# SamuelGong/FLASHE

Hardware: AMD Instinct MI355X
Metric: ciphertexts/sec (enc+agg+dec), 1e7-elem vector; achieved HBM GB/s fraction (higher is better)
Workload: dtype u128

## Files before the change

flashe_amd/csrc/device_common.h:

```cpp
#pragma once
#include "kernels.h"

#include <algorithm>
#include <cstdlib>
#include <vector>

#ifdef FLASHE_TUNING
#define FLASHE_TUNE_ENV(name) getenv(name)
#else
#define FLASHE_TUNE_ENV(name) (static_cast<const char *>(nullptr))
#endif

namespace flashe {

typedef unsigned __int128 u128;
typedef __attribute__((address_space(3))) uint32_t lds_u32;
typedef __attribute__((address_space(3))) uint8_t lds_u8;
typedef uint64_t u64x2 __attribute__((ext_vector_type(2)));

constexpr int kTabWords = 32768;
constexpr int kIterShiftWord = 1024;
constexpr int kPrfThreads = 1024;

#define SEL_B0 0x0c020400u
// ... 260 lines not shown
__device__ __forceinline__ CtrPrefix scalar_prefix(const CtrPrefix &c)
{
    return CtrPrefix{{static_cast<uint32_t>(__builtin_amdgcn_readfirstlane(c.u[0])), static_cast<uint32_t>(__builtin_amdgcn_readfirstlane(c.u[1])),
                      static_cast<uint32_t>(__builtin_amdgcn_readfirstlane(c.u[2])), static_cast<uint32_t>(__builtin_amdgcn_readfirstlane(c.u[3]))}};
}

__device__ __forceinline__ CtrUniform ctr_uniform(const RoundKeys &rk, const uint32_t *__restrict__ te4, const CtrPrefix &c, uint32_t x3)
{
    const uint32_t S1 = c.u[1] ^ te4[512 + ((x3 >> 8) & 0xffu)];
    const uint32_t S2 = c.u[2] ^ te4[256 + ((x3 >> 16) & 0xffu)];
    const uint32_t S3 = c.u[3] ^ te4[x3 >> 24];
    CtrUniform r;
    r.u[0] = te4[256 + ((S1 >> 16) & 0xffu)] ^ te4[512 + ((S2 >> 8) & 0xffu)] ^ te4[768 + (S3 & 0xffu)] ^ rk.w[8];
    r.u[1] = te4[S1 >> 24] ^ te4[256 + ((S2 >> 16) & 0xffu)] ^ te4[512 + ((S3 >> 8) & 0xffu)] ^ rk.w[9];
    r.u[2] = te4[S2 >> 24] ^ te4[256 + ((S3 >> 16) & 0xffu)] ^ te4[768 + (S1 & 0xffu)] ^ rk.w[10];
    r.u[3] = te4[S3 >> 24] ^ te4[512 + ((S1 >> 8) & 0xffu)] ^ te4[768 + (S2 & 0xffu)] ^ rk.w[11];
    return r;
}

__device__ __forceinline__ void ctr_round2(const LaneRegs lr, uint32_t c0, uint32_t v0, const CtrUniform &U, uint32_t (&s)[4])
{
    const uint32_t s0 = c0 ^ v0;
    s[0] = U.u[0] ^ T0(s0, SEL_B3);
    s[1] = U.u[1] ^ T3(s0, SEL_B0);
    s[2] = U.u[2] ^ T2(s0, SEL_B1);
    s[3] = U.u[3] ^ T1(s0, SEL_B2);
}

__device__ __forceinline__ u128 words_to_u128(const uint32_t (&s)[4])
{
    const uint64_t hi = (static_cast<uint64_t>(s[0]) << 32) | s[1];
    const uint64_t lo = (static_cast<uint64_t>(s[2]) << 32) | s[3];
    return (static_cast<u128>(hi) << 64) | lo;
}

__device__ __forceinline__ void set_block(uint32_t (&s)[4], uint32_t iter, uint32_t idx, uint64_t ctr)
{
    s[0] = iter; s[1] = idx; s[2] = static_cast<uint32_t>(ctr >> 32); s[3] = static_cast<uint32_t>(ctr);
}

__device__ __forceinline__ u128 ld128(const uint64_t *p)
{
    const ulonglong2 v = *reinterpret_cast<const ulonglong2 *>(p);
    return (static_cast<u128>(v.y) << 64) | v.x;
}
__device__ __forceinline__ void st128(uint64_t *p, u128 v)
{
    *reinterpret_cast<ulonglong2 *>(p) = make_ulonglong2(static_cast<uint64_t>(v), static_cast<uint64_t>(v >> 64));
}

#define FLASHE_GLOBAL(T, p) (reinterpret_cast<__attribute__((address_space(1))) T *>(reinterpret_cast<uintptr_t>(p)))
__device__ __forceinline__ uint32_t ld32_g(const uint32_t *p) { return *FLASHE_GLOBAL(const uint32_t, p); }
__device__ __forceinline__ uint64_t ld64_g(const uint64_t *p) { return *FLASHE_GLOBAL(const uint64_t, p); }
__device__ __forceinline__ uint64_t ld64_nt_g(const uint64_t *p) { return __builtin_nontemporal_load(FLASHE_GLOBAL(const uint64_t, p)); }
__device__ __forceinline__ u128 ld128_g(const uint64_t *p)
{
    const u64x2 v = *FLASHE_GLOBAL(const u64x2, p);
    return (static_cast<u128>(v[1]) << 64) | v[0];
}
__device__ __forceinline__ u128 ld128_nt_g(const uint64_t *p)
{
    const u64x2 v = __builtin_nontemporal_load(FLASHE_GLOBAL(const u64x2, p));
    return (static_cast<u128>(v[1]) << 64) | v[0];
}
__device__ __forceinline__ void st128_nt_g(uint64_t *p, u128 v)
{
    u64x2 r;
    r[0] = static_cast<uint64_t>(v); r[1] = static_cast<uint64_t>(v >> 64);
    __builtin_nontemporal_store(r, FLASHE_GLOBAL(u64x2, p));
}

__device__ __forceinline__ u128 ld128_nt(const uint64_t *p)
{
    const u64x2 v = __builtin_nontemporal_load(reinterpret_cast<const u64x2 *>(p));
    return (static_cast<u128>(v[1]) << 64) | v[0];
}
__device__ __forceinline__ void st128_nt(uint64_t *p, u128 v)
{
    u64x2 r;
    r[0] = static_cast<uint64_t>(v); r[1] = static_cast<uint64_t>(v >> 64);
    __builtin_nontemporal_store(r, reinterpret_cast<u64x2 *>(p));
}


__device__ __forceinline__ double u128_to_double(u128 v)
{
    const uint64_t hi = static_cast<uint64_t>(v >> 64), lo = static_cast<uint64_t>(v);
    if (hi == 0) return static_cast<double>(lo);
    const int sh = 64 - __clzll(static_cast<long long>(hi));
    uint64_t m = static_cast<uint64_t>(v >> sh);
    const u128 dropped = v & ((static_cast<u128>(1) << sh) - 1);
    if (dropped) m |= 1;
    return ldexp(static_cast<double>(m), sh);
}

template <typename T>
__device__ __forceinline__ uint64_t quantize_one(T v, T alpha, T scale, T den, double u)
{
#pragma clang fp contract(off)
    v = v < -alpha ? -alpha : (v > alpha ? alpha : v);
    v = v + alpha;
    v = v * scale;
    v = v / den;
    return static_cast<uint64_t>(static_cast<int64_t>(floor(static_cast<double>(v) + u)));
}

__device__ __forceinline__ const CodecLayer *codec_layer_of(const Codec &c, uint64_t key)
{
    int lo = 0, hi = c.n_layers - 1;
    while (lo < hi) {
        const int mid = (lo + hi + 1) >> 1;
        if (c.layers[mid].start <= key) lo = mid; else hi = mid - 1;
    }
    return c.layers + lo;
}

__device__ __forceinline__ uint64_t codec_quantize(const Codec &c, uint64_t k)
{
    if (c.layers != nullptr) {
        const uint64_t key = c.k0 + k;
        const CodecLayer *L = codec_layer_of(c, key);
        const uint64_t r = key - L->start;
        return L->x_is_f64 ? quantize_one<double>(*FLASHE_GLOBAL(const double, static_cast<const double *>(L->x) + r), L->p0, L->p1, L->p2, c.u[k])
                           : quantize_one<float>(*FLASHE_GLOBAL(const float, static_cast<const float *>(L->x) + r), static_cast<float>(L->p0),
                                                 static_cast<float>(L->p1), static_cast<float>(L->p2), c.u[k]);
    }
    return c.x_is_f64 ? quantize_one<double>(static_cast<const double *>(c.x)[k], c.alpha, c.scale, c.den, c.u[k])
                      : quantize_one<float>(static_cast<const float *>(c.x)[k], static_cast<float>(c.alpha), static_cast<float>(c.scale),
                                            static_cast<float>(c.den), c.u[k]);
}

__device__ __forceinline__ double codec_unquantize(const Codec &c, uint64_t k, u128 v)
{
#pragma clang fp contract(off)
    if (c.layers != nullptr) {
        const CodecLayer *L = codec_layer_of(c, c.k0 + k);
        return u128_to_double(v) * L->p1 / L->p2 - L->p0;
    }
    return u128_to_double(v) * c.two_a / c.uden - c.ac;
}


static inline void masks_of(int b, uint64_t *lo, uint64_t *hi)
{
    if (b >= 128) { *lo = ~0ull; *hi = ~0ull; }
    else if (b > 64) { *lo = ~0ull; *hi = (1ull << (b - 64)) - 1; }
    else if (b == 64) { *lo = ~0ull; *hi = 0; }
    else { *lo = (1ull << b) - 1; *hi = 0; }
}

static inline int grid_for(const LaunchEnv &env, uint64_t work_items, int threads)
{
    uint64_t blocks = (work_items + threads - 1) / threads;
    if (blocks < 1) blocks = 1;
    if (blocks > static_cast<uint64_t>(env.num_cus)) blocks = env.num_cus;
    return static_cast<int>(blocks);
}


constexpr int kStreamThreads = 256;

static inline int stream_grid(const LaunchEnv &env, uint64_t items)
{
    uint64_t blocks = (items + kStreamThreads - 1) / kStreamThreads;
    const uint64_t cap = static_cast<uint64_t>(env.num_cus) * 8;
    if (blocks > cap) blocks = cap;
// ... 6 lines not shown
```

flashe_amd/csrc/kernels.hip:

```cpp
#include "device_common.h"

namespace flashe {

struct IdxLists {
    uint32_t add[kMaxIdx];
    uint32_t minus[kMaxIdx];
};

struct PrfParams {
    const uint64_t *in;
    uint64_t *out;
    const uint32_t *te0;
    uint64_t n;
    uint64_t first, count;
    uint64_t blk_first, blk_count;
    uint64_t mask_lo, mask_hi;
    uint32_t iter;
    int in_limbs;
    int n_add, n_minus;
    uint32_t n_jobs;
    int b, m;
    Codec cq;
};

__global__ __launch_bounds__(kPrfThreads) void prf_wide_kernel(const RoundKeys rk, const PrfParams p, const IdxLists lists)
{
    const uint32_t iter = p.iter + p.te0[kIterShiftWord];
    __shared__ uint32_t tab[kTabWords];
    fill_tables(tab, p.te0);
    const LaneRegs lr = lane_regs(tab);
    const u128 mask = (static_cast<u128>(p.mask_hi) << 64) | p.mask_lo;

    for (uint64_t base = static_cast<uint64_t>(blockIdx.x) * kPrfThreads; base < p.count;
         base += static_cast<uint64_t>(gridDim.x) * kPrfThreads) {
        const uint64_t e = base + threadIdx.x;
        if (e >= p.count) continue;
        const uint64_t j = p.first + e;
        u128 acc = 0;
        if (p.cq.x) acc = codec_quantize(p.cq, e);
        else if (p.in) acc = p.in_limbs == 2 ? ld128(p.in + 2 * e) : static_cast<u128>(p.in[e]);
        {
            int k = 0;
            for (; k + 1 < p.n_add; k += 2) {
                uint32_t s[2][4];
                set_block(s[0], iter, lists.add[k], j);
                set_block(s[1], iter, lists.add[k + 1], j);
                aes256_encrypt<2>(rk, lr, s);
                acc += words_to_u128(s[0]);
                acc += words_to_u128(s[1]);
            }
            if (k < p.n_add) {
                uint32_t s[1][4];
                set_block(s[0], iter, lists.add[k], j);
                aes256_encrypt<1>(rk, lr, s);
                acc += words_to_u128(s[0]);
            }
            k = 0;
            for (; k + 1 < p.n_minus; k += 2) {
                uint32_t s[2][4];
                set_block(s[0], iter, lists.minus[k], j);
                set_block(s[1], iter, lists.minus[k + 1], j);
                aes256_encrypt<2>(rk, lr, s);
                acc -= words_to_u128(s[0]);
                acc -= words_to_u128(s[1]);
            }
            if (k < p.n_minus) {
                uint32_t s[1][4];
                set_block(s[0], iter, lists.minus[k], j);
                aes256_encrypt<1>(rk, lr, s);
                acc -= words_to_u128(s[0]);
            }
        }
        if (p.cq.fout) p.cq.fout[e] = codec_unquantize(p.cq, e, acc & mask);
        else st128(p.out + 2 * e, acc & mask);
    }
}

struct JobTable {
    uint32_t add[kMaxBatch], minus[kMaxBatch];
    uint64_t first[kMaxBatch], count[kMaxBatch];
    uint64_t big_end[kMaxBatch], small_end[kMaxBatch];
    const uint64_t *in[kMaxBatch];
    uint64_t *out[kMaxBatch];
// ... 90 lines not shown
        uint64_t *sum_out = tb.sum_out_of(v);
        const bool uni = FLASHE_CTR2 && epl == kBigEpl && ctr_fast && ((first + kw) & 255u) == 0;
        CtrUniform Ua{}, Ub{};
        if (uni) {
            const uint32_t x3 = static_cast<uint32_t>(first + kw) ^ rk.w[3];
            Ua = ctr_uniform(rk, te0, pre_a, x3);
            if (DBL) Ub = ctr_uniform(rk, te0, pre_b, x3);
        }
        for (int e = 0; e < epl; e++) {
            const uint64_t k = kw + static_cast<uint64_t>(e) * 64u + lane;
            if (k >= count) break;
            const uint64_t j = first + k;
            u128 acc = !in ? static_cast<u128>(0) : in_limbs == 2 ? ld128(in + 2 * k) : static_cast<u128>(in[k]);
            u64x2 held[KIND == 2 ? kSumRegs : 1];
            if (KIND == 2 && n_in > 1) {
#pragma unroll
                for (int c = 0; c < kSumRegs; c++) {
                    const int cc = c + 1 < n_in ? c + 1 : 0;
                    held[c] = __builtin_nontemporal_load(reinterpret_cast<const u64x2 *>(in + static_cast<uint64_t>(cc) * in_stride + 2 * k));
                }
                for (int c = kSumRegs + 1; c < n_in; c++) acc += ld128_nt(in + static_cast<uint64_t>(c) * in_stride + 2 * k);
            }
            uint32_t s[DBL ? 2 : 1][4];
            if (uni) {
                const uint32_t v0 = T3(static_cast<uint32_t>(j) ^ rk.w[3], SEL_B0);
                ctr_round2(lr, pre_a.u[0], v0, Ua, s[0]);
                if (DBL) ctr_round2(lr, pre_b.u[0], v0, Ub, s[DBL ? 1 : 0]);
                aes256_rounds<DBL ? 2 : 1, 3>(rk, lr, s, true);
            } else if (ctr_fast) {
                const CtrVar x = ctr_var(rk, lr, static_cast<uint32_t>(j));
                ctr_round1(pre_a, x, s[0]);
                if (DBL) ctr_round1(pre_b, x, s[DBL ? 1 : 0]);
                aes256_rounds<DBL ? 2 : 1, 2>(rk, lr, s, true);
            } else {
                set_block(s[0], iter, ia, j);
                if (DBL) set_block(s[DBL ? 1 : 0], iter, im, j);
                aes256_encrypt<DBL ? 2 : 1>(rk, lr, s);
            }
            if (KIND == 2 && n_in > 1) {
#pragma unroll
                for (int c = 0; c < kSumRegs; c++)
                    if (c + 1 < n_in) acc += (static_cast<u128>(held[c][1]) << 64) | held[c][0];
                acc &= mask;
                if (sum_out) st128_nt(sum_out + 2 * k, acc);
            }
            acc += words_to_u128(s[0]);
            if (DBL) acc -= words_to_u128(s[DBL ? 1 : 0]);
            if (KIND == 2) st128_nt(out + 2 * k, acc & mask);
            else st128(out + 2 * k, acc & mask);
        }
    }
}

#ifndef FLASHE_HALF_U
#define FLASHE_HALF_U 1
#endif
constexpr int kMaxChains = 16;
constexpr int kMaxLinks = 128;
struct ChainTable {
    uint64_t first[kMaxChains], count[kMaxChains];
    uint64_t wend[kMaxChains];
    uint16_t link0[kMaxChains], sbase[kMaxChains];
    uint8_t len[kMaxChains];
    uint8_t flags[kMaxChains];
    uint32_t idx[kMaxLinks + kMaxChains];
    const uint64_t *in[kMaxLinks];
    uint64_t *out[kMaxLinks];
    uint64_t *sum_out[kMaxChains];
};

__device__ __forceinline__ CtrPrefix load_prefix(const uint32_t *pre_lds, int s)
{
    const uint4 v = *reinterpret_cast<const uint4 *>(pre_lds + 4 * s);
    return CtrPrefix{{static_cast<uint32_t>(__builtin_amdgcn_readfirstlane(v.x)), static_cast<uint32_t>(__builtin_amdgcn_readfirstlane(v.y)),
                      static_cast<uint32_t>(__builtin_amdgcn_readfirstlane(v.z)), static_cast<uint32_t>(__builtin_amdgcn_readfirstlane(v.w))}};
}

__device__ __forceinline__ void loads_landed(const u128 &a, const u128 &b)
{
    asm volatile("" ::"v"(static_cast<uint64_t>(a)), "v"(static_cast<uint64_t>(a >> 64)), "v"(static_cast<uint64_t>(b)),
                 "v"(static_cast<uint64_t>(b >> 64)));
}

template <class T> __device__ __forceinline__ void swap_regs(T &a, T &b) { const T t = a; a = b; b = t; }

__device__ __forceinline__ uint64_t uniform64(uint64_t v)
{
    return static_cast<uint32_t>(__builtin_amdgcn_readfirstlane(static_cast<uint32_t>(v))) |
           (static_cast<uint64_t>(static_cast<uint32_t>(__builtin_amdgcn_readfirstlane(static_cast<uint32_t>(v >> 32)))) << 32);
}

template <int THREADS, bool SUM, bool CODEC>
__global__ __launch_bounds__(THREADS) void prf_chain_kernel(const RoundKeys rk, const ChainTable tb, int n_chains, int all_half_arg,
                                                              uint32_t iter0, uint64_t mask_lo, uint64_t mask_hi,
                                                              const uint32_t *__restrict__ te0, const Codec cq)
{
    constexpr bool DMASK = false;
    uint64_t *const dmask = nullptr;
#include "prf_chain_body.inc"
}

template <int THREADS>
__global__ __launch_bounds__(THREADS) void prf_chain_dmask_kernel(const RoundKeys rk, const ChainTable tb, int n_chains, int all_half_arg,
                                                                    uint32_t iter0, uint64_t mask_lo, uint64_t mask_hi,
                                                                    const uint32_t *__restrict__ te0, uint64_t *__restrict__ dmask)
{
    constexpr bool SUM = true, CODEC = false, DMASK = true;
    const Codec cq{};
#include "prf_chain_body.inc"
}

__device__ __forceinline__ uint64_t extract64(u128 S, int sh)
{
    return sh >= 128 ? 0ull : static_cast<uint64_t>(S >> sh);
}

constexpr int kSmallThreads = 1024;
constexpr int kTch = 8;

__global__ __launch_bounds__(kSmallThreads) void prf_small_kernel(const RoundKeys rk, const PrfParams p, const IdxLists lists)
{
    const uint32_t iter = p.iter + p.te0[kIterShiftWord];
    __shared__ uint32_t tab[kTabWords];
    fill_tables(tab, p.te0);
    const LaneRegs lr = lane_regs(tab);

    const uint64_t J = p.n_jobs, d = p.n / J, r = p.n % J;
    const uint64_t m = static_cast<uint64_t>(p.m);
    const uint64_t nb1 = (d + 1 + m - 1) / m;
    const uint64_t nb0 = d ? (d + m - 1) / m : 0;
    const uint64_t range_end = p.first + p.count;

    for (uint64_t Bl = static_cast<uint64_t>(blockIdx.x) * kSmallThreads + threadIdx.x; Bl < p.blk_count;
         Bl += static_cast<uint64_t>(gridDim.x) * kSmallThreads) {
        const uint64_t B = p.blk_first + Bl;
        uint64_t begin, len, i;
        if (B < r * nb1) {
            const uint64_t c = B / nb1;
            i = B - c * nb1; begin = c * (d + 1); len = d + 1;
        } else {
            const uint64_t B2 = B - r * nb1, c = B2 / nb0;
            i = B2 - c * nb0; begin = r * (d + 1) + c * d; len = d;
        }
        const uint64_t j0 = begin + i * m;
        const uint64_t rem = len - i * m;
        const int cnt = rem < m ? static_cast<int>(rem) : static_cast<int>(m);
        const uint64_t ctr = begin + i;

        for (int t0 = 0; t0 < cnt; t0 += kTch) {
            uint64_t acc[kTch];
#pragma unroll
            for (int u = 0; u < kTch; u++) {
                const uint64_t j = j0 + t0 + u;
                const bool on = t0 + u < cnt && j >= p.first && j < range_end;
                acc[u] = !on ? 0ull : p.cq.x ? codec_quantize(p.cq, j - p.first) : p.in ? p.in[j - p.first] : 0ull;
            }
            int k = 0;
            for (; k + 1 < p.n_add; k += 2) {
                uint32_t s[2][4];
                set_block(s[0], iter, lists.add[k], ctr);
                set_block(s[1], iter, lists.add[k + 1], ctr);
                aes256_encrypt<2>(rk, lr, s);
                const u128 S0 = words_to_u128(s[0]), S1 = words_to_u128(s[1]);
#pragma unroll
                for (int u = 0; u < kTch; u++) acc[u] += extract64(S0, p.b * (t0 + u)) + extract64(S1, p.b * (t0 + u));
            }
            if (k < p.n_add) {
                uint32_t s[1][4];
                set_block(s[0], iter, lists.add[k], ctr);
                aes256_encrypt<1>(rk, lr, s);
                const u128 S0 = words_to_u128(s[0]);
#pragma unroll
                for (int u = 0; u < kTch; u++) acc[u] += extract64(S0, p.b * (t0 + u));
            }
            k = 0;
            for (; k + 1 < p.n_minus; k += 2) {
                uint32_t s[2][4];
                set_block(s[0], iter, lists.minus[k], ctr);
                set_block(s[1], iter, lists.minus[k + 1], ctr);
                aes256_encrypt<2>(rk, lr, s);
                const u128 S0 = words_to_u128(s[0]), S1 = words_to_u128(s[1]);
#pragma unroll
                for (int u = 0; u < kTch; u++) acc[u] -= extract64(S0, p.b * (t0 + u)) + extract64(S1, p.b * (t0 + u));
            }
            if (k < p.n_minus) {
                uint32_t s[1][4];
                set_block(s[0], iter, lists.minus[k], ctr);
                aes256_encrypt<1>(rk, lr, s);
                const u128 S0 = words_to_u128(s[0]);
#pragma unroll
// ... 1363 lines not shown
    return launch_prf_chains(env, iter, static_cast<int>(chains.size()), chains.data(), n, n_jobs);
}

hipError_t launch_prf_jobs(const LaunchEnv &env, uint32_t iter, bool dbl, int n_entries, const PrfJob *jobs, uint64_t n, uint32_t n_jobs)
{
    {
        const hipError_t e = launch_jobs_as_chains(env, iter, dbl, n_entries, jobs, n, n_jobs);
        if (e != hipErrorNotSupported) return e;
    }
    if (env.codec && env.b > 64) return hipErrorNotSupported;
    if (n_entries > kMaxBatch) {
        const int launches = (n_entries + kMaxBatch - 1) / kMaxBatch, per = (n_entries + launches - 1) / launches;
        for (int e0 = 0; e0 < n_entries; e0 += per) {
            const hipError_t e = launch_prf_jobs(env, iter, dbl, std::min(per, n_entries - e0), jobs + e0, n, n_jobs);
            if (e != hipSuccess) return e;
        }
        return hipSuccess;
    }
    if (env.elem32) return hipErrorInvalidValue;
    if (env.b <= 64) return launch_prf_jobs_small(env, iter, dbl, n_entries, jobs, n, n_jobs);
    if (lone_small_double_job(env, dbl, n_entries, jobs)) {
        constexpr int kLatThreads = 256;
        JobTable tb{};
        tb.add[0] = jobs[0].add_idx; tb.minus[0] = jobs[0].minus_idx; tb.first[0] = jobs[0].first; tb.count[0] = jobs[0].count;
        tb.in[0] = jobs[0].in_dev; tb.out[0] = jobs[0].out_dev; tb.in_limbs[0] = static_cast<uint8_t>(jobs[0].in_limbs); tb.n_in[0] = 1;
        tb.big_end[0] = 0; tb.small_end[0] = (jobs[0].count + kLatThreads - 1) / kLatThreads;
        uint64_t lo, hi;
        masks_of(env.b, &lo, &hi);
        const uint64_t cus = static_cast<uint64_t>(env.num_cus);
        const int grid = static_cast<int>(tb.small_end[0] < cus ? tb.small_end[0] : cus);
        hipLaunchKernelGGL((prf_wide_batch_kernel<true, kLatThreads, 3, JobTable>), dim3(grid), dim3(kLatThreads), 0, env.stream, env.rk, tb, 1, n, iter, lo,
                           hi, env.te0_dev);
        return hipGetLastError();
    }
    JobTable tb{};
    int nv = 0;
    uint64_t big[kMaxBatch];
    uint64_t n_big = 0;
    constexpr uint64_t kBigTile = static_cast<uint64_t>(kPrfThreads) * kBigEpl;
    for (int e = 0; e < n_entries; e++) {
        if (jobs[e].count == 0) continue;
        tb.add[nv] = jobs[e].add_idx; tb.minus[nv] = jobs[e].minus_idx;
        tb.first[nv] = jobs[e].first; tb.count[nv] = jobs[e].count;
        tb.in[nv] = jobs[e].in_dev; tb.out[nv] = jobs[e].out_dev; tb.in_limbs[nv] = static_cast<uint8_t>(jobs[e].in_limbs);
        if (jobs[e].n_in > 255 || (jobs[e].n_in > 1 && (jobs[e].in_limbs != 2 || !jobs[e].in_dev))) return hipErrorInvalidValue;
        tb.n_in[nv] = static_cast<uint8_t>(jobs[e].n_in ? jobs[e].n_in : 1); tb.in_stride[nv] = jobs[e].in_stride;
        tb.sum_out[nv] = jobs[e].n_in > 1 ? jobs[e].sum_out_dev : nullptr;
        big[nv] = jobs[e].count / kBigTile;
        n_big += big[nv++];
    }
    if (nv == 0) return hipSuccess;
    const uint64_t cus = static_cast<uint64_t>(env.num_cus);
    uint64_t excess = n_big % cus;
    for (int v = nv - 1; v >= 0 && excess; v--) {
        const uint64_t take = big[v] < excess ? big[v] : excess;
        big[v] -= take; excess -= take;
    }
    uint64_t be = 0, se = 0;
    for (int v = 0; v < nv; v++) {
        be += big[v];
        se += (tb.count[v] - big[v] * kBigTile + kPrfThreads - 1) / kPrfThreads;
        tb.big_end[v] = be; tb.small_end[v] = se;
    }
    const uint64_t tiles = be + se;
    uint64_t lo, hi;
    masks_of(env.b, &lo, &hi);
    const int grid = static_cast<int>(tiles < cus ? tiles : cus);
#define JOBS_LAUNCH(DBL, MULTI)                                                                                              \
    hipLaunchKernelGGL((prf_wide_batch_kernel<DBL, kPrfThreads, MULTI, JobTable>), dim3(grid), dim3(kPrfThreads), 0, env.stream, env.rk, tb, \
                       nv, n, iter, lo, hi, env.te0_dev)
    bool summed = false;
    for (int v = 0; v < nv; v++) summed |= tb.n_in[v] > 1;
    if (dbl) { if (summed) JOBS_LAUNCH(true, 2); else if (nv > 1) JOBS_LAUNCH(true, 1); else JOBS_LAUNCH(true, 0); }
    else { if (summed) JOBS_LAUNCH(false, 2); else if (nv > 1) JOBS_LAUNCH(false, 1); else JOBS_LAUNCH(false, 0); }
#undef JOBS_LAUNCH
    return hipGetLastError();
}

static hipError_t launch_small_chains(const LaunchEnv &env, uint32_t iter, int n_chains, const PrfChain *chains, uint64_t n, uint32_t n_jobs);

#ifndef FLASHE_CHAIN_QUARTER_DEFAULT
#define FLASHE_CHAIN_QUARTER_DEFAULT 1
#endif
hipError_t launch_prf_chains(const LaunchEnv &env, uint32_t iter, int n_chains, const PrfChain *chains, uint64_t n, uint32_t n_jobs)
{
    if (env.b <= 64) return launch_small_chains(env, iter, n_chains, chains, n, n_jobs);
    struct Piece { const PrfChain *ch; int l0, l1; uint64_t tiles; };
    std::vector<Piece> pieces;
    uint64_t total_tiles = 0;
    bool summed = false;
    uint64_t *dmask = nullptr;
    for (int i = 0; i < n_chains; i++) {
        const PrfChain &c = chains[i];
        if (c.dmask_dev && (n_chains != 1 || !c.sum_out_dev || c.single)) return hipErrorInvalidValue;
        dmask = c.dmask_dev;
        if (c.count == 0 || c.n_out == 0) continue;
        if (((c.first + c.count - 1) >> 32) != (c.first >> 32)) return hipErrorNotSupported;
        if (c.sum_out_dev) { if (c.n_out > kMaxLinks) return hipErrorNotSupported; summed = true; }
        const uint64_t tiles = (c.first + c.count - (c.first & ~255ull) + 255) / 256;
        pieces.push_back(Piece{&c, 0, c.n_out, tiles});
        total_tiles += tiles;
    }
    if (pieces.empty()) return hipSuccess;
    const uint64_t waves = static_cast<uint64_t>(env.num_cus) * (kPrfThreads / 64);
    bool all_half = total_tiles < 2 * waves;
    static const bool tune = FLASHE_TUNE_ENV("FLASHE_CHAIN_TUNE") != nullptr;
    int force_parts = 0, force_grid = 0, probe = 0;
    if (tune) {
        if (const char *e = FLASHE_TUNE_ENV("FLASHE_CHAIN_HALF")) all_half = atoi(e) != 0;
        if (const char *e = FLASHE_TUNE_ENV("FLASHE_CHAIN_PARTS")) force_parts = atoi(e);
        if (const char *e = FLASHE_TUNE_ENV("FLASHE_CHAIN_GRID")) force_grid = atoi(e);
        if (const char *e = FLASHE_TUNE_ENV("FLASHE_CHAIN_PROBE")) probe = atoi(e) == 1 ? 0x100 : atoi(e) == 2 ? 0x200 : 0;
    }
    bool only_single = true;
    for (const Piece &pc : pieces) only_single &= pc.ch->single && !pc.ch->sum_out_dev;
    int single_parts = 0;
    if (only_single && all_half && !force_parts && !(tune && FLASHE_TUNE_ENV("FLASHE_CHAIN_HALF"))) {
        single_parts = static_cast<int>(std::min<uint64_t>((2 * waves + total_tiles - 1) / total_tiles, kMaxChains / pieces.size()));
        if (single_parts < 1) single_parts = 1;
        uint64_t cut_tiles = 0;
        for (const Piece &pc : pieces) cut_tiles += pc.tiles * static_cast<uint64_t>(std::min(single_parts, pc.l1));
        all_half = 2 * cut_tiles < waves;
    }
    uint64_t cuttable_tiles = 0, fixed_items = 0;
    for (const Piece &pc : pieces) {
        if (pc.l1 >= 8 && !pc.ch->sum_out_dev) cuttable_tiles += pc.tiles;
        else fixed_items += 2 * pc.tiles;
    }
    bool quarter = !env.codec && !summed && !single_parts && all_half && 4 * total_tiles <= waves && !force_parts && FLASHE_CHAIN_QUARTER_DEFAULT;
    if (tune) {
        if (const char *e = FLASHE_TUNE_ENV("FLASHE_CHAIN_QUARTER")) quarter = atoi(e) != 0 && !env.codec && !summed && !single_parts && all_half;
    }
    std::vector<Piece> cut;
    for (const Piece &pc : pieces) {
        int parts = (pc.l1 + kMaxLinks - 1) / kMaxLinks;
        if (single_parts) {
            parts = std::max(parts, std::min(single_parts, pc.l1));
        } else if (quarter && !pc.ch->sum_out_dev && pc.l1 >= 2) {
            uint64_t cut4 = 0, fixed4 = 0;
            for (const Piece &o : pieces) (o.l1 >= 2 && !o.ch->sum_out_dev ? cut4 : fixed4) += 4 * o.tiles;
            const uint64_t want = fixed4 < waves ? std::max<uint64_t>((waves - fixed4) / cut4, 1) : 1;
            parts = std::max<int>(parts, static_cast<int>(std::min<uint64_t>(want, static_cast<uint64_t>(pc.l1))));
            parts = std::min(parts, std::max(1, kMaxChains / static_cast<int>(pieces.size())));
            parts = std::max(parts, (pc.l1 + kMaxLinks - 1) / kMaxLinks);
        } else if (all_half && 2 * total_tiles < waves && !pc.ch->sum_out_dev) {
            const uint64_t aim = waves + waves * 15 / 100;
            const uint64_t want = fixed_items < aim && cuttable_tiles ? (aim - fixed_items + cuttable_tiles) / (2 * cuttable_tiles) : 1;
            const int cap = std::max(1, pc.l1 / 4);
            parts = std::max<int>(parts, static_cast<int>(std::min<uint64_t>(want, static_cast<uint64_t>(cap))));
            parts = std::min(parts, std::max(1, kMaxChains / static_cast<int>(pieces.size())));
            parts = std::max(parts, (pc.l1 + kMaxLinks - 1) / kMaxLinks);
        }
        if (force_parts > 0 && !pc.ch->sum_out_dev) parts = std::max(std::min(force_parts, pc.l1), (pc.l1 + kMaxLinks - 1) / kMaxLinks);
        for (int k = 0; k < parts; k++) {
            const int a = static_cast<int>(static_cast<int64_t>(pc.l1) * k / parts), b = static_cast<int>(static_cast<int64_t>(pc.l1) * (k + 1) / parts);
            if (b > a) cut.push_back(Piece{pc.ch, a, b, pc.tiles});
        }
    }
    uint64_t lo, hi;
    masks_of(env.b, &lo, &hi);
    size_t at = 0;
    while (at < cut.size()) {
        ChainTable tb{};
        int nc = 0, links = 0, streams = 0;
        uint64_t wend = 0, tiles = 0;
        while (at < cut.size() && nc < kMaxChains && links + (cut[at].l1 - cut[at].l0) <= kMaxLinks) {
            const Piece &pc = cut[at++];
            const PrfChain &c = *pc.ch;
            const int len = pc.l1 - pc.l0, ns = len + (c.single ? 0 : 1);
            tb.first[nc] = c.first; tb.count[nc] = c.count;
            tb.link0[nc] = static_cast<uint16_t>(links); tb.sbase[nc] = static_cast<uint16_t>(streams);
            tb.len[nc] = static_cast<uint8_t>(len);
            tb.flags[nc] = static_cast<uint8_t>((c.single ? 1 : 0) | (c.in_limbs == 2 ? 2 : 0));
            tb.sum_out[nc] = c.sum_out_dev;
            for (int s = 0; s < ns; s++) tb.idx[streams + s] = c.idx[pc.l0 + s];
            for (int l = 0; l < len; l++) {
                tb.in[links + l] = c.in_dev ? c.in_dev[pc.l0 + l] : nullptr;
                tb.out[links + l] = c.out_dev[pc.l0 + l];
            }
            wend += pc.tiles * static_cast<uint64_t>(ns);
            tb.wend[nc] = wend;
            tiles += pc.tiles;
            links += len; streams += ns; nc++;
        }
        const uint64_t items = quarter ? 4 * tiles : all_half ? 2 * tiles : tiles, cus = static_cast<uint64_t>(env.num_cus);
        int grid = static_cast<int>(items < cus ? items : cus);
        if (force_grid > 0) grid = force_grid;
        Codec cq{};
        if (env.codec) {
            if (cut.size() != 1 || cut[0].l1 - cut[0].l0 != 1) return hipErrorInvalidValue;
            cq = *env.codec;
        }
        if (env.codec && summed) return hipErrorInvalidValue;
        if (dmask)
            hipLaunchKernelGGL((prf_chain_dmask_kernel<kPrfThreads>), dim3(grid), dim3(kPrfThreads), 0, env.stream, env.rk, tb, nc,
                               (all_half ? 1 : 0) | (quarter ? 4 : 0) | probe, iter, lo, hi, env.te0_dev, dmask);
        else if (env.codec)
            hipLaunchKernelGGL((prf_chain_kernel<kPrfThreads, false, true>), dim3(grid), dim3(kPrfThreads), 0, env.stream, env.rk, tb, nc,
                               (all_half ? 1 : 0) | (quarter ? 4 : 0) | probe, iter, lo, hi, env.te0_dev, cq);
        else if (summed)
            hipLaunchKernelGGL((prf_chain_kernel<kPrfThreads, true, false>), dim3(grid), dim3(kPrfThreads), 0, env.stream, env.rk, tb, nc,
                               (all_half ? 1 : 0) | (quarter ? 4 : 0) | probe, iter, lo, hi, env.te0_dev, cq);
        else
            hipLaunchKernelGGL((prf_chain_kernel<kPrfThreads, false, false>), dim3(grid), dim3(kPrfThreads), 0, env.stream, env.rk, tb, nc,
                               (all_half ? 1 : 0) | (quarter ? 4 : 0) | probe, iter, lo, hi, env.te0_dev, cq);
        const hipError_t e = hipGetLastError();
        if (e != hipSuccess) return e;
    }
    return hipSuccess;
}

static SmallParams small_params_of(const LaunchEnv &env, uint32_t iter, uint64_t n, uint32_t n_jobs)
{
    SmallParams p{};
    p.n = n; p.n_jobs = n_jobs; p.iter = iter; p.b = env.b; p.m = 128 / env.b; p.te0 = env.te0_dev;
    { static const int v = FLASHE_TUNE_ENV("FLASHE_SMALL_DIRECT") ? atoi(FLASHE_TUNE_ENV("FLASHE_SMALL_DIRECT")) : 1; p.no_direct = v == 0 ? 1 : v == 2 ? 2 : 0; }
    { static const int v = FLASHE_TUNE_ENV("FLASHE_SMALL_FIXED") ? atoi(FLASHE_TUNE_ENV("FLASHE_SMALL_FIXED")) : 1; p.no_fixed_width = v == 0; }
    p.m_magic = static_cast<uint32_t>(((1ull << 32) + p.m - 1) / p.m);
    uint64_t hi;
    masks_of(env.b, &p.mask_lo, &hi);
    unsigned __int128 top = 0;
    for (int t = 0; t < p.m; t++) top |= static_cast<unsigned __int128>(1) << (env.b * t + env.b - 1);
    p.top_lo = static_cast<uint64_t>(top); p.top_hi = static_cast<uint64_t>(top >> 64);
    const uint64_t mm = p.m, d = n / n_jobs, nb1 = (d + 1 + mm - 1) / mm, nb0 = d ? (d + mm - 1) / mm : 0;
    p.nb1_magic = nb1 > 1 && nb1 < (1ull << 32) ? static_cast<uint32_t>((1ull << 32) / nb1) : 0;
    p.nb0_magic = nb0 > 1 && nb0 < (1ull << 32) ? static_cast<uint32_t>((1ull << 32) / nb0) : 0;
    return p;
}

hipError_t launch_small_reduce_decrypt(const LaunchEnv &env, uint32_t iter, uint32_t add_idx, bool has_minus, uint32_t minus_idx, uint64_t n,
                                       uint32_t n_jobs, uint64_t first, uint64_t count, int C, const uint64_t *const *ops, uint64_t *agg_out_dev,
                                       uint64_t *out_dev, int out_elem_bytes)
{
    if (env.b > 64 || env.codec || n >= (1ull << 32) || n == 0 || n_jobs == 0 || C < 1 || C > kMaxOps) return hipErrorNotSupported;
    if ((env.elem32 || out_elem_bytes == 4) && env.b > 32) return hipErrorInvalidValue;
    if (out_elem_bytes != 8 && !(out_elem_bytes == 4 && env.elem32)) return hipErrorInvalidValue;
    if (env.prf_backend != PRF_AUTO && env.prf_backend != PRF_TABLE) return hipErrorNotSupported;
    if (count == 0) return hipSuccess;
    SmallParams p = small_params_of(env, iter, n, n_jobs);
    p.swp_prio = 1;
    const uint64_t bf = block_of(first, n, n_jobs, p.m), bc = block_of(first + count - 1, n, n_jobs, p.m) - bf + 1;
    PtrTable t;
    for (int c = 0; c < kMaxOps; c++) t.p[c] = c < C ? ops[c] : nullptr;
    const uint64_t tiles = (bc + 63) / 64, groups = (tiles + kSmallThreads / 64 - 1) / (kSmallThreads / 64), cus = static_cast<uint64_t>(env.num_cus);
    const int grid = static_cast<int>(groups < cus ? groups : cus);
    int cb = C < 2 ? 1 : 2;
    { static const int force = FLASHE_TUNE_ENV("FLASHE_SMALL_REDUCE_CB") ? atoi(FLASHE_TUNE_ENV("FLASHE_SMALL_REDUCE_CB")) : 0; if (force >= 1) cb = force; }
    static const int probe = FLASHE_TUNE_ENV("FLASHE_SMALL_REDUCE_PROBE") ? 0x100 : 0;
#define SRD_LAUNCH(CB)                                                                                                                      \
    hipLaunchKernelGGL((small_reduce_decrypt_kernel<CB, 2>), dim3(grid), dim3(kSmallThreads), 0, env.stream, env.rk, p, add_idx, minus_idx, \
                       (has_minus ? 1 : 0) | probe, first, count, bf, bc, C, t, agg_out_dev, out_dev)
    static const bool split_off = FLASHE_TUNE_ENV("FLASHE_SMALL_REDUCE_SPLIT") && atoi(FLASHE_TUNE_ENV("FLASHE_SMALL_REDUCE_SPLIT")) == 0;
    if (env.b <= 32 && !split_off) {
        const uint64_t tiles32 = (bc + 31) / 32, groups32 = (tiles32 + kSmallThreads / 64 - 1) / (kSmallThreads / 64);
        const int grid32 = static_cast<int>(groups32 < cus ? groups32 : cus);
        uintptr_t low_bits = reinterpret_cast<uintptr_t>(out_dev) | reinterpret_cast<uintptr_t>(agg_out_dev);
        for (int c = 0; c < C; c++) low_bits |= reinterpret_cast<uintptr_t>(ops[c]);
        static const bool quad_off = FLASHE_TUNE_ENV("FLASHE_SMALL_REDUCE_QUAD") && atoi(FLASHE_TUNE_ENV("FLASHE_SMALL_REDUCE_QUAD")) == 0;
        int quad = (low_bits & 15u) == 0 && !quad_off ? 0x200 : 0;
        if (quad && env.elem32) {
            const uint32_t tile_elems = 32u * static_cast<uint32_t>(p.m);
            uint32_t best = 4;
            double best_util = 0.0;
            for (uint32_t e : {4u, 3u, 2u}) {
                if (tile_elems % e) continue;
                const uint32_t lanes = tile_elems / e;
                const double util = static_cast<double>(lanes) / (64.0 * ((lanes + 63u) / 64u));
                if (util > best_util + 1e-9) { best_util = util; best = e; }
            }
            static const int force_e = FLASHE_TUNE_ENV("FLASHE_SMALL_REDUCE_EPL") ? atoi(FLASHE_TUNE_ENV("FLASHE_SMALL_REDUCE_EPL")) : 0;
            if (force_e >= 2 && force_e <= 4 && tile_elems % static_cast<uint32_t>(force_e) == 0) best = static_cast<uint32_t>(force_e);
            quad |= static_cast<int>(best & 3u) << 10;
        }
#define SRDS_LAUNCH(CB, IT, OT)                                                                                                               \
    hipLaunchKernelGGL((small_reduce_decrypt_split_kernel<CB, IT, OT>), dim3(grid32), dim3(kSmallThreads), 0, env.stream, env.rk, p, add_idx,  \
                       minus_idx, (has_minus ? 1 : 0) | probe | quad, first, count, bf, bc, C, t, agg_out_dev, out_dev)
#define SRDS_PICK(CB)                                                                                                                          \
// ... 255 lines not shown
```

flashe_amd/csrc/prf_chain_body.inc:

```
    static_assert(!DMASK || (SUM && !CODEC), "the decrypt mask is written by summed chains only");
    (void)dmask;
    const uint32_t iter = iter0 + te0[kIterShiftWord];
    constexpr uint32_t WAVES = THREADS / 64;
    __shared__ uint32_t tab[kTabWords];
    __shared__ __attribute__((aligned(16))) uint32_t pre_lds[(kMaxLinks + kMaxChains) * 4];
    __shared__ uint64_t d_tlo[kMaxChains], d_cend[kMaxChains];
    int all_half = all_half_arg;
    fill_tables(tab, te0);
#ifdef FLASHE_TUNING
    if (all_half & 0x100) return;
#endif
    const LaneRegs lr = lane_regs(tab);
    const u128 mask = (static_cast<u128>(mask_hi) << 64) | mask_lo;
    {
        const int last = n_chains - 1;
        const int n_streams = tb.sbase[last] + tb.len[last] + ((tb.flags[last] & 1) ? 0 : 1);
        for (int s = threadIdx.x; s < n_streams; s += THREADS) {
            int i = 0;
            while (i < last && s >= tb.sbase[i + 1]) i++;
            const CtrPrefix c = ctr_prefix(rk, lr, iter, tb.idx[s], static_cast<uint32_t>(tb.first[i] >> 32));
            *reinterpret_cast<uint4 *>(pre_lds + 4 * s) = make_uint4(c.u[0], c.u[1], c.u[2], c.u[3]);
        }
        if (threadIdx.x < static_cast<unsigned>(n_chains)) {
            const int i = threadIdx.x;
            const uint64_t Wt = tb.wend[last], cw = i ? tb.wend[i - 1] : 0;
            const uint32_t w = tb.len[i] + ((tb.flags[i] & 1) ? 0u : 1u);
            uint64_t a, b, T;
            if (Wt <= 0xffffffffull && gridDim.x <= 0xffffu) {
                const uint32_t W32 = static_cast<uint32_t>(Wt), G = gridDim.x, g = blockIdx.x, c32 = static_cast<uint32_t>(cw);
                const uint32_t q = W32 / G, r = W32 % G;
                const uint32_t lo = q * g + r * g / G, hi = q * (g + 1) + r * (g + 1) / G;
                const uint32_t T32 = (static_cast<uint32_t>(tb.wend[i]) - c32) / w;
                const uint32_t a32 = lo > c32 ? (lo - c32 + w - 1) / w : 0, b32 = hi > c32 ? (hi - c32 + w - 1) / w : 0;
                T = T32; a = a32; b = b32;
            } else {
                const uint64_t G = gridDim.x, g = blockIdx.x;
                const uint64_t lo = Wt / G * g + (Wt % G) * g / G, hi = Wt / G * (g + 1) + (Wt % G) * (g + 1) / G;
                T = (tb.wend[i] - cw) / w;
                a = lo > cw ? (lo - cw + w - 1) / w : 0; b = hi > cw ? (hi - cw + w - 1) / w : 0;
            }
            if (a > T) a = T;
            if (b > T) b = T;
            d_tlo[i] = a; d_cend[i] = b - a;
        }
        __syncthreads();
        if (threadIdx.x == 0) {
            uint64_t acc = 0;
            for (int i = 0; i < n_chains; i++) { acc += d_cend[i]; d_cend[i] = acc; }
        }
        __syncthreads();
    }
#ifdef FLASHE_TUNING
    if (all_half & 0x200) return;
#endif
    const bool quarter = !CODEC && !SUM && (all_half & 4) != 0;
    all_half &= 1;
    const uint32_t wave = static_cast<uint32_t>(__builtin_amdgcn_readfirstlane(threadIdx.x >> 6));
    const uint32_t lane = threadIdx.x & 63u;
    const uint64_t Ng = uniform64(d_cend[n_chains - 1]);
    const uint64_t n_full = (all_half || quarter) ? 0 : Ng - Ng % WAVES;
    const uint64_t n_items = quarter ? 4 * Ng : n_full + 2 * (Ng - n_full);
    int cur = 0;
    uint64_t cbeg = 0;
    for (uint64_t q = wave; q < n_items; q += WAVES) {
        const bool whole = q < n_full;
        const uint64_t L = quarter ? (q >> 2) : whole ? q : n_full + ((q - n_full) >> 1);
        const uint32_t half = whole || quarter ? 0u : static_cast<uint32_t>((q - n_full) & 1u);
        while (L >= uniform64(d_cend[cur])) cbeg = uniform64(d_cend[cur++]);
        const uint64_t first = tb.first[cur], end = first + tb.count[cur];
        const uint64_t tj = (first & ~255ull) + 256u * (uniform64(d_tlo[cur]) + (L - cbeg)) + 128u * half +
                            (quarter ? 64u * static_cast<uint32_t>(q & 3u) : 0u);
        const int link0 = tb.link0[cur], sbase = tb.sbase[cur];
        const bool single = tb.flags[cur] & 1, in2 = tb.flags[cur] & 2;
        const int n_streams = tb.len[cur] + (single ? 0 : 1);
        if (whole) {
            const uint32_t x3 = static_cast<uint32_t>(tj) ^ rk.w[3];
            const uint32_t jl = static_cast<uint32_t>(tj) + lane;
            uint32_t vA0 = T3(jl ^ rk.w[3], SEL_B0), vA1 = T3((jl + 64u) ^ rk.w[3], SEL_B0);
            uint32_t vB0 = T3((jl + 128u) ^ rk.w[3], SEL_B0), vB1 = T3((jl + 192u) ^ rk.w[3], SEL_B0);
            u128 pA0 = 0, pA1 = 0, pB0 = 0, pB1 = 0;
            u128 qA0 = 0, qA1 = 0, qB0 = 0, qB1 = 0;
            u128 dA0 = 0, dA1 = 0, dB0 = 0, dB1 = 0;
            uint64_t *const sum_out = SUM ? tb.sum_out[cur] : nullptr;
            for (int c = 0; c < n_streams; c++) {
                const CtrPrefix pre = load_prefix(pre_lds, sbase + c);
                const CtrUniform U = ctr_uniform(rk, te0, pre, x3);
                const int link = single ? c : c - 1;
                const uint64_t *in = link >= 0 ? tb.in[link0 + link] : nullptr;
                uint64_t *out = link >= 0 ? tb.out[link0 + link] : nullptr;
                const bool last_stream = c == n_streams - 1;
#pragma unroll 1
                for (int p = 0; p < 2; p++) {
                    const uint64_t jb = tj + 128u * p;
                    if (jb < end && jb + 128u > first) {
                        const uint64_t j0 = jb + lane, j1 = j0 + 64u, k0 = j0 - first, k1 = j1 - first;
                        const bool a0 = j0 >= first && j0 < end, a1 = j1 >= first && j1 < end;
                        u128 x0 = 0, x1 = 0;
                        if (CODEC && cq.x != nullptr && link >= 0) {
                            if (a0) x0 = codec_quantize(cq, k0);
                            if (a1) x1 = codec_quantize(cq, k1);
                        } else if (in != nullptr && in2) {
                            if (a0) x0 = ld128(in + 2 * k0);
                            if (a1) x1 = ld128(in + 2 * k1);
                        } else if (in != nullptr) {
                            if (a0) x0 = static_cast<u128>(in[k0]);
                            if (a1) x1 = static_cast<u128>(in[k1]);
                        }
                        uint32_t s[2][4];
                        ctr_round2(lr, pre.u[0], vA0, U, s[0]);
                        ctr_round2(lr, pre.u[0], vA1, U, s[1]);
                        aes256_rounds<2, 3>(rk, lr, s, true);
                        loads_landed(x0, x1);
                        const u128 c0 = words_to_u128(s[0]), c1 = words_to_u128(s[1]);
                        const u128 r0 = x0 + (single ? c0 : pA0 - c0), r1 = x1 + (single ? c1 : pA1 - c1);
                        if (CODEC && cq.fout != nullptr) {
                            if (a0 && link >= 0) cq.fout[k0] = codec_unquantize(cq, k0, r0 & mask);
                            if (a1 && link >= 0) cq.fout[k1] = codec_unquantize(cq, k1, r1 & mask);
                        } else {
                            if (a0 && out != nullptr) st128(out + 2 * k0, r0 & mask);
                            if (a1 && out != nullptr) st128(out + 2 * k1, r1 & mask);
                        }
                        if constexpr (SUM) {
                            if (link >= 0) {
                                if (p == 0) { qA0 += r0; qA1 += r1; } else { qB0 += r0; qB1 += r1; }
                            }
                            if (last_stream && sum_out != nullptr) {
                                if (p == 0) {
                                    if (a0) st128_nt(sum_out + 2 * k0, qA0 & mask);
                                    if (a1) st128_nt(sum_out + 2 * k1, qA1 & mask);
                                } else {
                                    if (a0) st128_nt(sum_out + 2 * k0, qB0 & mask);
                                    if (a1) st128_nt(sum_out + 2 * k1, qB1 & mask);
                                }
                            }
                        }
                        if constexpr (DMASK) {
                            if (c == 0) {
                                if (p == 0) { dA0 = c0; dA1 = c1; } else { dB0 = c0; dB1 = c1; }
                            }
                            if (last_stream) {
                                if (p == 0) {
                                    if (a0) st128_nt(dmask + 2 * k0, (c0 - dA0) & mask);
                                    if (a1) st128_nt(dmask + 2 * k1, (c1 - dA1) & mask);
                                } else {
                                    if (a0) st128_nt(dmask + 2 * k0, (c0 - dB0) & mask);
                                    if (a1) st128_nt(dmask + 2 * k1, (c1 - dB1) & mask);
                                }
                            }
                        }
                        pA0 = c0; pA1 = c1;
                    }
                    swap_regs(pA0, pB0); swap_regs(pA1, pB1); swap_regs(vA0, vB0); swap_regs(vA1, vB1);
                }
            }
        } else if (quarter) {
            if (!CODEC && !SUM && tj < end && tj + 64u > first) {
                const uint64_t j0 = tj + lane, k0 = j0 - first;
// ... 98 lines not shown
```

Before: 68.35 billion.

## Add specialised 128-bit decrypt-mask sum chain kernel using buffer loads/stores

Adds a dedicated kernel for the 128-bit, full-mask, single-chain decrypt-mask summed case. It reads 64-bit inputs through buffer resources, accumulates the running sum in 96 bits instead of full 128-bit adds, and writes outputs with 128-bit buffer stores, with separate edge and interior tile paths. The goal is to cut address arithmetic and ALU work, and to issue wider, non-temporal stores for the mask and sum outputs. It adds a new code path gated on shape checks and a count limit, which raises code size and the maintenance burden.

```diff
diff --git a/flashe_amd/csrc/device_common.h b/flashe_amd/csrc/device_common.h
--- a/flashe_amd/csrc/device_common.h
+++ b/flashe_amd/csrc/device_common.h
@@ -366,6 +366,25 @@
     __builtin_nontemporal_store(r, reinterpret_cast<u64x2 *>(p));
 }
 
+typedef uint32_t u32x2 __attribute__((ext_vector_type(2)));
+typedef uint32_t u32x4 __attribute__((ext_vector_type(4)));
+__device__ __forceinline__ __amdgpu_buffer_rsrc_t buf_rsrc(const void *p, uint32_t bytes)
+{
+    const uint64_t a = reinterpret_cast<uintptr_t>(p);
+    const uint64_t u = static_cast<uint32_t>(__builtin_amdgcn_readfirstlane(static_cast<uint32_t>(a))) |
+                       (static_cast<uint64_t>(static_cast<uint32_t>(__builtin_amdgcn_readfirstlane(static_cast<uint32_t>(a >> 32)))) << 32);
+    return __builtin_amdgcn_make_buffer_rsrc(reinterpret_cast<void *>(u), 0, static_cast<int>(__builtin_amdgcn_readfirstlane(bytes)), 0x00020000);
+}
+__device__ __forceinline__ uint64_t buf_ld64(__amdgpu_buffer_rsrc_t r, uint32_t voff)
+{
+    const u32x2 v = __builtin_amdgcn_raw_buffer_load_b64(r, voff, 0, 0);
+    return (static_cast<uint64_t>(v.y) << 32) | v.x;
+}
+template <int AUX = 0> __device__ __forceinline__ void buf_st128(__amdgpu_buffer_rsrc_t r, uint32_t voff, u128 v)
+{
+    const u32x4 w = {static_cast<uint32_t>(v), static_cast<uint32_t>(v >> 32), static_cast<uint32_t>(v >> 64), static_cast<uint32_t>(v >> 96)};
+    __builtin_amdgcn_raw_buffer_store_b128(w, r, voff, 0, AUX);
+}
 
 __device__ __forceinline__ double u128_to_double(u128 v)
 {
diff --git a/flashe_amd/csrc/kernels.hip b/flashe_amd/csrc/kernels.hip
--- a/flashe_amd/csrc/kernels.hip
+++ b/flashe_amd/csrc/kernels.hip
@@ -1,4 +1,5 @@
 #include "device_common.h"
+#include <type_traits>
 
 namespace flashe {
 
@@ -255,7 +256,15 @@
                  "v"(static_cast<uint64_t>(b >> 64)));
 }
 
+__device__ __forceinline__ void loads_landed(const uint64_t &a, const uint64_t &b)
+{
+    asm volatile("" ::"v"(a), "v"(b));
+}
+
 template <class T> __device__ __forceinline__ void swap_regs(T &a, T &b) { const T t = a; a = b; b = t; }
+
+__device__ __forceinline__ void add96(uint64_t &lo, uint32_t &hi, uint64_t x) { lo += x; hi += lo < x ? 1u : 0u; }
+__device__ __forceinline__ u128 join96(uint64_t lo, uint32_t hi) { return (static_cast<u128>(hi) << 64) | lo; }
 
 __device__ __forceinline__ uint64_t uniform64(uint64_t v)
 {
@@ -268,7 +277,7 @@
                                                               uint32_t iter0, uint64_t mask_lo, uint64_t mask_hi,
                                                               const uint32_t *__restrict__ te0, const Codec cq)
 {
-    constexpr bool DMASK = false;
+    constexpr bool DMASK = false, D128 = false;
     uint64_t *const dmask = nullptr;
 #include "prf_chain_body.inc"
 }
@@ -278,7 +287,21 @@
                                                                     uint32_t iter0, uint64_t mask_lo, uint64_t mask_hi,
                                                                     const uint32_t *__restrict__ te0, uint64_t *__restrict__ dmask)
 {
-    constexpr bool SUM = true, CODEC = false, DMASK = true;
+    constexpr bool SUM = true, CODEC = false, DMASK = true, D128 = false;
+    const Codec cq{};
+#include "prf_chain_body.inc"
+}
+
+#ifndef FLASHE_SUM128
+#define FLASHE_SUM128 1
+#endif
+constexpr uint64_t kSum128MaxCount = 0x0fffff00ull;
+template <int THREADS>
+__global__ __launch_bounds__(THREADS) void prf_dmask_sum128_kernel(const RoundKeys rk, const ChainTable tb, int n_chains, int all_half_arg,
+                                                                     uint32_t iter0, uint64_t mask_lo, uint64_t mask_hi,
+                                                                     const uint32_t *__restrict__ te0, uint64_t *__restrict__ dmask)
+{
+    constexpr bool SUM = true, CODEC = false, DMASK = true, D128 = true;
     const Codec cq{};
 #include "prf_chain_body.inc"
 }
@@ -1808,6 +1831,14 @@
 #ifndef FLASHE_CHAIN_QUARTER_DEFAULT
 #define FLASHE_CHAIN_QUARTER_DEFAULT 1
 #endif
+static bool sum128_shape(const LaunchEnv &env, int nc, const ChainTable &tb, uint64_t lo, uint64_t hi)
+{
+    if (env.b != 128 || ~lo != 0 || ~hi != 0 || nc != 1 || (tb.flags[0] & 3) != 0 || !tb.sum_out[0] || tb.count[0] > kSum128MaxCount) return false;
+    for (int l = 0; l < tb.len[0]; l++)
+        if (!tb.in[tb.link0[0] + l] || !tb.out[tb.link0[0] + l]) return false;
+    return true;
+}
+
 hipError_t launch_prf_chains(const LaunchEnv &env, uint32_t iter, int n_chains, const PrfChain *chains, uint64_t n, uint32_t n_jobs)
 {
     if (env.b <= 64) return launch_small_chains(env, iter, n_chains, chains, n, n_jobs);
@@ -1918,7 +1949,10 @@
             cq = *env.codec;
         }
         if (env.codec && summed) return hipErrorInvalidValue;
-        if (dmask)
+        if (dmask && FLASHE_SUM128 && sum128_shape(env, nc, tb, lo, hi))
+            hipLaunchKernelGGL((prf_dmask_sum128_kernel<kPrfThreads>), dim3(grid), dim3(kPrfThreads), 0, env.stream, env.rk, tb, nc,
+                               (all_half ? 1 : 0) | (quarter ? 4 : 0) | probe, iter, lo, hi, env.te0_dev, dmask);
+        else if (dmask)
             hipLaunchKernelGGL((prf_chain_dmask_kernel<kPrfThreads>), dim3(grid), dim3(kPrfThreads), 0, env.stream, env.rk, tb, nc,
                                (all_half ? 1 : 0) | (quarter ? 4 : 0) | probe, iter, lo, hi, env.te0_dev, dmask);
         else if (env.codec)
diff --git a/flashe_amd/csrc/prf_chain_body.inc b/flashe_amd/csrc/prf_chain_body.inc
--- a/flashe_amd/csrc/prf_chain_body.inc
+++ b/flashe_amd/csrc/prf_chain_body.inc
@@ -1,4 +1,5 @@
     static_assert(!DMASK || (SUM && !CODEC), "the decrypt mask is written by summed chains only");
+    static_assert(!D128 || DMASK, "the int_bits = 128 specialisation is the decrypt-mask chain's");
     (void)dmask;
     const uint32_t iter = iter0 + te0[kIterShiftWord];
     constexpr uint32_t WAVES = THREADS / 64;
@@ -11,7 +12,7 @@
     if (all_half & 0x100) return;
 #endif
     const LaneRegs lr = lane_regs(tab);
-    const u128 mask = (static_cast<u128>(mask_hi) << 64) | mask_lo;
+    const u128 mask = D128 ? ~static_cast<u128>(0) : (static_cast<u128>(mask_hi) << 64) | mask_lo;
     {
         const int last = n_chains - 1;
         const int n_streams = tb.sbase[last] + tb.len[last] + ((tb.flags[last] & 1) ? 0 : 1);
@@ -71,8 +72,14 @@
         const uint64_t tj = (first & ~255ull) + 256u * (uniform64(d_tlo[cur]) + (L - cbeg)) + 128u * half +
                             (quarter ? 64u * static_cast<uint32_t>(q & 3u) : 0u);
         const int link0 = tb.link0[cur], sbase = tb.sbase[cur];
-        const bool single = tb.flags[cur] & 1, in2 = tb.flags[cur] & 2;
+        const bool single = !D128 && (tb.flags[cur] & 1), in2 = !D128 && (tb.flags[cur] & 2);
         const int n_streams = tb.len[cur] + (single ? 0 : 1);
+        if constexpr (D128) {
+            if (whole) {
+#include "prf_chain_sum128_tile.inc"
+                continue;
+            }
+        }
         if (whole) {
             const uint32_t x3 = static_cast<uint32_t>(tj) ^ rk.w[3];
             const uint32_t jl = static_cast<uint32_t>(tj) + lane;
diff --git a/flashe_amd/csrc/prf_chain_sum128_tile.inc b/flashe_amd/csrc/prf_chain_sum128_tile.inc
--- /dev/null
+++ b/flashe_amd/csrc/prf_chain_sum128_tile.inc
@@ -0,0 +1,75 @@
+{
+    const uint32_t cnt = static_cast<uint32_t>(tb.count[cur]);
+    const uint32_t k0 = static_cast<uint32_t>(tj - first) + lane;
+    const uint32_t v8 = 8u * k0, v16 = 16u * k0;
+    const uint32_t x3 = static_cast<uint32_t>(tj) ^ rk.w[3];
+    const uint32_t jl = static_cast<uint32_t>(tj) + lane;
+    const auto tile = [&](auto edge_tag) {
+        constexpr bool EDGE = decltype(edge_tag)::value;
+        const uint32_t vA0 = T3(jl ^ rk.w[3], SEL_B0), vA1 = T3((jl + 64u) ^ rk.w[3], SEL_B0);
+        const uint32_t vB0 = T3((jl + 128u) ^ rk.w[3], SEL_B0), vB1 = T3((jl + 192u) ^ rk.w[3], SEL_B0);
+        const auto live = [&](int p) { const uint64_t jb = tj + 128u * p; return !EDGE || (jb < end && jb + 128u > first); };
+        const auto blocks = [&](int p, const CtrPrefix &pre, const CtrUniform &U, u128 &c0, u128 &c1) {
+            uint32_t w0, w1;
+            if (p == 0) { w0 = vA0; w1 = vA1; } else { w0 = vB0; w1 = vB1; }
+            uint32_t s[2][4];
+            ctr_round2(lr, pre.u[0], w0, U, s[0]);
+            ctr_round2(lr, pre.u[0], w1, U, s[1]);
+            aes256_rounds<2, 3>(rk, lr, s, true);
+            c0 = words_to_u128(s[0]); c1 = words_to_u128(s[1]);
+        };
+        u128 fA0 = 0, fA1 = 0, fB0 = 0, fB1 = 0;
+        {
+            const CtrPrefix pre = load_prefix(pre_lds, sbase);
+            const CtrUniform U = ctr_uniform(rk, te0, pre, x3);
+#pragma unroll 1
+            for (int p = 0; p < 2; p++) {
+                if (live(p)) {
+                    u128 c0, c1;
+                    blocks(p, pre, U, c0, c1);
+                    if (p == 0) { fA0 = c0; fA1 = c1; } else { fB0 = c0; fB1 = c1; }
+                }
+            }
+        }
+        u128 pA0 = fA0, pA1 = fA1, pB0 = fB0, pB1 = fB1;
+        uint64_t sA0 = 0, sA1 = 0, sB0 = 0, sB1 = 0;
+        uint32_t hA0 = 0, hA1 = 0, hB0 = 0, hB1 = 0;
+        const auto rsum = buf_rsrc(tb.sum_out[cur], 16u * cnt), rdm = buf_rsrc(dmask, 16u * cnt);
+        for (int c = 1; c < n_streams; c++) {
+            const CtrPrefix pre = load_prefix(pre_lds, sbase + c);
+            const CtrUniform U = ctr_uniform(rk, te0, pre, x3);
+            const auto rin = buf_rsrc(tb.in[link0 + c - 1], 8u * cnt), rout = buf_rsrc(tb.out[link0 + c - 1], 16u * cnt);
+            const bool last_stream = c == n_streams - 1;
+#pragma unroll 1
+            for (int p = 0; p < 2; p++) {
+                if (live(p)) {
+                    const uint32_t o8 = v8 + 1024u * p, o16 = v16 + 2048u * p;
+                    bool a0 = true, a1 = true;
+                    if constexpr (EDGE) { a0 = k0 + 128u * p < cnt; a1 = k0 + 128u * p + 64u < cnt; }
+                    uint64_t x0 = 0, x1 = 0;
+                    if (a0) x0 = buf_ld64(rin, o8);
+                    if (a1) x1 = buf_ld64(rin, o8 + 512u);
+                    u128 c0, c1;
+                    blocks(p, pre, U, c0, c1);
+                    loads_landed(x0, x1);
+                    const auto finish = [&](u128 &p0, u128 &p1, uint64_t &s0, uint32_t &h0, uint64_t &s1, uint32_t &h1, const u128 &f0,
+                                            const u128 &f1) {
+                        if (a0) buf_st128(rout, o16, x0 + (p0 - c0));
+                        if (a1) buf_st128(rout, o16 + 1024u, x1 + (p1 - c1));
+                        add96(s0, h0, x0); add96(s1, h1, x1);
+                        if (last_stream) {
+                            const u128 d0 = c0 - f0, d1 = c1 - f1;
+                            if (a0) { buf_st128<2>(rdm, o16, d0); buf_st128<2>(rsum, o16, join96(s0, h0) - d0); }
+                            if (a1) { buf_st128<2>(rdm, o16 + 1024u, d1); buf_st128<2>(rsum, o16 + 1024u, join96(s1, h1) - d1); }
+                        }
+                        p0 = c0; p1 = c1;
+                    };
+                    if (p == 0) finish(pA0, pA1, sA0, hA0, sA1, hA1, fA0, fA1);
+                    else finish(pB0, pB1, sB0, hB0, sB1, hB1, fB0, fB1);
+                }
+            }
+        }
+    };
+    if (tj < first || tj + 256u > end) tile(std::true_type{});
+    else tile(std::false_type{});
+}
```

New measurement: 70.40 billion (median of 6 runs). 3.0% higher.
